# CVlab315/Domain-Adaptative-Hand-Pose-Estimation

Measured on AMD Instinct MI355X. Metric: images/sec (unique source+target images per A+B+C training iteration, 2*B*N/t_iter), higher is better.
Workload: dtype bf16; 1 GPU; RHD->H3D domain-adaptation iteration (steps A+B+C), resnet50 + 3-deconv neck + main head + 3 adversarial multiscale-fusion heads, 256x256, batch 64 source + 64 target per GPU, random init, synthetic batches; arch=resnet50, image_size=256, per_gpu_batch=64, global_batch=64, parallelism=dp1, hip_graphs=True, gradient_exchange=none (one rank)

## Files before the change

### domain-adaptative-hand-pose-estimation_amd/csrc/bn.hip

```cpp
#include "common.h"
#include "fp8_common.h"
#include <stdlib.h>
#include <string>

struct BnPlan { int cpr, TX, TY, colgroups, nslices, rows_per_slice; };

static BnPlan bn_plan(long rows, int C, int CH, long slice_cap_override = 0) {
  BnPlan p; p.cpr = C / CH;
  p.TX = p.cpr < 256 ? p.cpr : 256;
  while (256 % p.TX) --p.TX;
  p.TY = 256 / p.TX;
  p.colgroups = cdiv(p.cpr, p.TX);
  long want = rows / ((long)p.TY * 8); if (want < 1) want = 1;
  static const long slice_cap = getenv("MI355_BN_SLICES") ? atol(getenv("MI355_BN_SLICES")) : 1024;
  long cap = (slice_cap_override ? slice_cap_override : slice_cap) / p.colgroups; if (cap < 1) cap = 1;
  if (want > cap) want = cap;
  long rps = (rows + want - 1) / want; rps = ((rps + p.TY - 1) / p.TY) * p.TY;
  p.rows_per_slice = (int)rps; p.nslices = (int)((rows + rps - 1) / rps);
  return p;
}

static long bwd_slices() { static const long v = getenv("MI355_BN_BWD_SLICES") ? atol(getenv("MI355_BN_BWD_SLICES")) : 768; return v; }
extern "C" size_t mi355_bn_workspace(long rows, int C) {
  int ns = 0;
// ... 299 lines not shown
#pragma unroll
    for (int j = 0; j < 16; ++j) { s1 += q1[j]; s2 += q2[j]; }
  }
#pragma unroll
  for (int o = 32; o > 0; o >>= 1) { s1 += __shfl_down(s1, o, 64); s2 += __shfl_down(s2, o, 64); }
  if (lane != 0) return;
  if (dbeta) dbeta[c] = db0 + s1;
  if (dgamma) dgamma[c] = dg0 + s2;
  if (coeff) { coeff[c] = g * is; coeff[C + c] = s1 * inv_rows; coeff[2 * C + c] = s2 * inv_rows; }
}

template <typename T, int RELU, bool Q8 = false>
__global__ __launch_bounds__(256) void bn_bwd_apply_kernel(const T* __restrict__ dy, const T* __restrict__ x, const T* __restrict__ y,
                                                            const float* __restrict__ mean, const float* __restrict__ invstd,
                                                            const float* __restrict__ coeff, const float* __restrict__ beta,
                                                            T* __restrict__ dx, T* __restrict__ dres,
                                                            long rows, int C, int TX, const unsigned char* __restrict__ mask,
                                                            unsigned char* __restrict__ q8 = nullptr, float* __restrict__ q8_state = nullptr) {
  constexpr int CH = Chunk<T>::N;
  constexpr int relu = RELU;
  static_assert(!Q8 || CH == 8, "fp8 side output: bf16 gradients only");
  const int TY = 256 / TX;
  const int tx = threadIdx.x % TX, ty = threadIdx.x / TX;
  const int chunk = blockIdx.x * TX + tx;
  const bool colok = chunk * CH < C;
  if (!colok && !Q8) return;
  const int cpr = C / CH;
  float k0[CH], k1[CH], k2[CH], mu[CH], is[CH], sh[CH];
#pragma unroll
  for (int e = 0; e < CH; ++e) {
    const int c = colok ? chunk * CH + e : 0;
    k0[e] = coeff[c]; k1[e] = coeff[C + c]; k2[e] = coeff[2 * C + c]; mu[e] = mean[c]; is[e] = invstd[c];
    sh[e] = (relu == 2) ? beta[c] - mu[e] * k0[e] : 0.f;
  }
  float qscale = 0.f, amax = 0.f; unsigned seen = 0;
  if constexpr (Q8) { qscale = q8_state[0]; seen = fp8_amax_seen(q8_state); }
  auto finish = [&](size_t off, float (&g)[CH], float (&v)[CH], const float (&o)[CH], unsigned mb) {
    if (relu == 1) {
#pragma unroll
      for (int e = 0; e < CH; ++e) g[e] = o[e] > 0.f ? g[e] : 0.f; }
    else if (relu == 3) {
#pragma unroll
      for (int e = 0; e < CH; ++e) g[e] = ((mb >> e) & 1u) ? g[e] : 0.f; }
    else if (relu == 2) {
#pragma unroll
      for (int e = 0; e < CH; ++e) g[e] = (v[e] * k0[e] + sh[e]) > 0.f ? g[e] : 0.f; }
    if (dres) Chunk<T>::store(dres + off, g);
#pragma unroll
    for (int e = 0; e < CH; ++e) v[e] = k0[e] * (g[e] - k1[e] - (v[e] - mu[e]) * is[e] * k2[e]);
    Chunk<T>::store(dx + off, v);
    if constexpr (Q8) {
      float w[8];
#pragma unroll
      for (int e = 0; e < 8; ++e) { w[e] = (float)(T)v[e]; amax = fmaxf(amax, fabsf(w[e])); }
      const uint2 o = pack8_fp8<true>(w, qscale);
      const unsigned nx = __shfl_down(o.x, 1, 64), ny = __shfl_down(o.y, 1, 64);
      if ((tx & 1) == 0) *reinterpret_cast<uint4*>(q8 + off) = make_uint4(o.x, o.y, nx, ny);
    }
  };
  const long stride = (long)gridDim.y * TY;
  long r = colok ? (long)blockIdx.y * TY + ty : rows;
  for (; r + stride < rows; r += 2 * stride) {
    const size_t off0 = (size_t)r * C + (size_t)chunk * CH, off1 = (size_t)(r + stride) * C + (size_t)chunk * CH;
    float g0[CH], v0[CH], o0[CH], g1[CH], v1[CH], o1[CH];
    Chunk<T>::load(dy + off0, g0); Chunk<T>::load(x + off0, v0);
    Chunk<T>::load(dy + off1, g1); Chunk<T>::load(x + off1, v1);
    if (relu == 1) { Chunk<T>::load(y + off0, o0); Chunk<T>::load(y + off1, o1); }
    unsigned m0 = 0, m1 = 0;
    if (relu == 3) { m0 = mask[(size_t)r * cpr + chunk]; m1 = mask[(size_t)(r + stride) * cpr + chunk]; }
    finish(off0, g0, v0, o0, m0); finish(off1, g1, v1, o1, m1);
  }
  if (r < rows) {
    const size_t off = (size_t)r * C + (size_t)chunk * CH;
    float g[CH], v[CH], o[CH]; Chunk<T>::load(dy + off, g); Chunk<T>::load(x + off, v);
    if (relu == 1) Chunk<T>::load(y + off, o);
    finish(off, g, v, o, relu == 3 ? (unsigned)mask[(size_t)r * cpr + chunk] : 0u);
  }
  if constexpr (Q8) fp8_record_amax(amax, q8_state, seen);
}

struct BnResArgs {
  const void* dy; const void* x; const float* mean; const float* invstd; const float* gamma; const float* beta;
  void* dx; void* dres; float* dgamma; float* dbeta; const unsigned char* mask;
  float* partial;
  long rows; int C, G, R, rpb, keep, accumulate; float inv_rows;
  unsigned spin_limit;
};
#define BN_RES_MAXBLK 1024
#define BN_RES_KR 0
#define BN_RES_NT 1024
__device__ unsigned long long bn_res_sync[BN_RES_MAXBLK + 1];
__device__ unsigned bn_res_err[4];

__device__ __forceinline__ bool bn_res_grid_barrier(unsigned nblk, int t, unsigned spin_limit, int* ok_lds) {
  asm volatile("s_waitcnt vmcnt(0)" ::: "memory");
  __syncthreads();
  if (t == 0) {
    int ok = 1;
    unsigned long long* st = bn_res_sync + nblk;
    const unsigned long long v = __hip_atomic_fetch_add(st, 1ull, __ATOMIC_RELAXED, __HIP_MEMORY_SCOPE_AGENT);
    const unsigned long long target = (v / nblk + 1ull) * nblk;
    if (v + 1ull != target) {
      unsigned spins = 0;
      while (__hip_atomic_load(st, __ATOMIC_RELAXED, __HIP_MEMORY_SCOPE_AGENT) < target) {
        __builtin_amdgcn_s_sleep(4);
        if (++spins > spin_limit) {
          __hip_atomic_fetch_add(bn_res_err, 1u, __ATOMIC_RELAXED, __HIP_MEMORY_SCOPE_AGENT);
          ok = 0;
          break;
        }
      }
    }
    *ok_lds = ok;
  }
  __syncthreads();
  return *ok_lds != 0;
}

template <typename T, int RELU, int KR, int NT>
__global__ __launch_bounds__(NT) void bn_bwd_resident_kernel(BnResArgs p) {
  constexpr int CH = Chunk<T>::N, GC = 8 * CH, RL = NT / 8, NW = NT / 64, NL = NT / (GC * 2), RR = KR * RL;
  extern __shared__ __attribute__((aligned(16))) char smem[];
  const int t = threadIdx.x, tx = t & 7, ty = t >> 3, lane = t & 63, wave = t >> 6;
  const int g = blockIdx.x % p.G, r = blockIdx.x / p.G;
  const long row0 = (long)r * p.rpb;
  long row1 = row0 + p.rpb; if (row1 > p.rows) row1 = p.rows;
  const int nrows = row1 > row0 ? (int)(row1 - row0) : 0;
  const int keep = p.keep;
  uint4* xs = reinterpret_cast<uint4*>(smem);
  uint4* ds = xs + (size_t)keep * 8;
  float* red = reinterpret_cast<float*>(ds + (size_t)keep * 8);
  float* tot = red + NW * GC * 2;
  int* bar_ok = reinterpret_cast<int*>(tot + GC * 2);
  const T* __restrict__ X = reinterpret_cast<const T*>(p.x);
  const T* __restrict__ DY = reinterpret_cast<const T*>(p.dy);
  const int C = p.C, cpr = C / CH, c0 = g * GC + tx * CH, chunk = c0 / CH;
  float mu[CH], is[CH], sc[CH], sft[CH], s1[CH], s2[CH];
#pragma unroll
  for (int e = 0; e < CH; ++e) {
    mu[e] = p.mean[c0 + e]; is[e] = p.invstd[c0 + e]; s1[e] = 0.f; s2[e] = 0.f;
    sc[e] = p.gamma[c0 + e] * is[e];
    sft[e] = (RELU == 2) ? p.beta[c0 + e] - mu[e] * sc[e] : 0.f;
  }
  auto mask_of = [&](int lr) -> unsigned { return (RELU == 3) ? (unsigned)p.mask[(size_t)(row0 + lr) * cpr + chunk] : 0u; };
  auto fold = [&](const uint4& qxv, const uint4& qdv, unsigned mb) {
    float v[CH], gq[CH]; Chunk<T>::unpack(qxv, v); Chunk<T>::unpack(qdv, gq);
#pragma unroll
    for (int e = 0; e < CH; ++e) {
      if (RELU == 2) gq[e] = (v[e] * sc[e] + sft[e]) > 0.f ? gq[e] : 0.f;
      if (RELU == 3) gq[e] = ((mb >> e) & 1u) ? gq[e] : 0.f;
      s1[e] += gq[e]; s2[e] += gq[e] * ((v[e] - mu[e]) * is[e]);
    }
  };
  uint4 rx[KR > 0 ? KR : 1], rd[KR > 0 ? KR : 1];
  {
    unsigned mk[KR > 0 ? KR : 1];
#pragma unroll
    for (int k = 0; k < KR; ++k) {
      const int lr = ty + k * RL;
      rx[k] = make_uint4(0, 0, 0, 0); rd[k] = make_uint4(0, 0, 0, 0); mk[k] = 0;
      if (lr < nrows) {
        const size_t off = (size_t)(row0 + lr) * C + c0;
        rx[k] = *reinterpret_cast<const uint4*>(X + off); rd[k] = *reinterpret_cast<const uint4*>(DY + off); mk[k] = mask_of(lr);
      }
    }
#pragma unroll
    for (int k = 0; k < KR; ++k)
      if (ty + k * RL < nrows) fold(rx[k], rd[k], mk[k]);
  }
  for (int base = RR + ty; base < nrows; base += 4 * RL) {
    uint4 qx[4], qd[4]; unsigned mk[4];
#pragma unroll
    for (int k = 0; k < 4; ++k) {
      const int lr = base + k * RL;
      if (lr < nrows) {
        const size_t off = (size_t)(row0 + lr) * C + c0;
        qx[k] = *reinterpret_cast<const uint4*>(X + off); qd[k] = *reinterpret_cast<const uint4*>(DY + off); mk[k] = mask_of(lr);
      }
    }
#pragma unroll
    for (int k = 0; k < 4; ++k) {
      const int lr = base + k * RL, li = lr - RR;
      if (lr < nrows) {
        if (li < keep) { xs[li * 8 + tx] = qx[k]; ds[li * 8 + tx] = qd[k]; }
        fold(qx[k], qd[k], mk[k]);
      }
    }
  }
#pragma unroll
  for (int o = 8; o < 64; o <<= 1) {
#pragma unroll
    for (int e = 0; e < CH; ++e) { s1[e] += __shfl_xor(s1[e], o, 64); s2[e] += __shfl_xor(s2[e], o, 64); }
  }
  if (lane < 8) {
#pragma unroll
    for (int e = 0; e < CH; ++e) { red[(wave * GC + tx * CH + e) * 2] = s1[e]; red[(wave * GC + tx * CH + e) * 2 + 1] = s2[e]; }
  }
  __syncthreads();
  float* part = p.partial + ((size_t)g * p.R) * (GC * 2);
  if (t < GC * 2) {
    float a = 0.f;
#pragma unroll
    for (int w = 0; w < NW; ++w) a += red[w * GC * 2 + t];
    __hip_atomic_store(part + (size_t)r * (GC * 2) + t, a, __ATOMIC_RELAXED, __HIP_MEMORY_SCOPE_AGENT);
  }
  const bool exchanged = bn_res_grid_barrier((unsigned)(p.G * p.R), t, p.spin_limit, bar_ok);
  {
    const int i = t % (GC * 2), s = t / (GC * 2);
    const __amdgpu_buffer_rsrc_t rs = __builtin_amdgcn_make_buffer_rsrc(part, 0, (unsigned)(p.R * GC * 2 * 4), 0x00020000);
    float a = 0.f;
    for (int rr0 = s; rr0 < p.R; rr0 += 8 * NL) {
      float q[8];
#pragma unroll
      for (int k = 0; k < 8; ++k) {
        const int rr = rr0 + k * NL;
        q[k] = rr < p.R ? __uint_as_float(__builtin_amdgcn_raw_buffer_load_b32(rs, (rr * (GC * 2) + i) * 4, 0, 16)) : 0.f;
      }
#pragma unroll
      for (int k = 0; k < 8; ++k) a += q[k];
    }
    red[s * GC * 2 + i] = a;
  }
  __syncthreads();
  if (t < GC * 2) {
    float a = 0.f;
#pragma unroll
    for (int s = 0; s < NL; ++s) a += red[s * GC * 2 + t];
    tot[t] = a;
  }
  __syncthreads();
  float k1[CH], k2[CH];
#pragma unroll
  for (int e = 0; e < CH; ++e) {
    s1[e] = tot[(tx * CH + e) * 2]; s2[e] = tot[(tx * CH + e) * 2 + 1];
    if (!exchanged) { s1[e] = __builtin_nanf(""); s2[e] = __builtin_nanf(""); }
    k1[e] = s1[e] * p.inv_rows; k2[e] = s2[e] * p.inv_rows;
  }
  if (r == 0 && ty == 0) {
#pragma unroll
    for (int e = 0; e < CH; ++e) {
      if (p.dbeta) p.dbeta[c0 + e] = (p.accumulate ? p.dbeta[c0 + e] : 0.f) + s1[e];
      if (p.dgamma) p.dgamma[c0 + e] = (p.accumulate ? p.dgamma[c0 + e] : 0.f) + s2[e];
    }
  }
  T* __restrict__ DX = reinterpret_cast<T*>(p.dx);
  T* __restrict__ DR = reinterpret_cast<T*>(p.dres);
  auto finish = [&](int lr, const uint4& qxv, const uint4& qdv, unsigned mb) {
    const size_t off = (size_t)(row0 + lr) * C + c0;
    float v[CH], gq[CH]; Chunk<T>::unpack(qxv, v); Chunk<T>::unpack(qdv, gq);
#pragma unroll
    for (int e = 0; e < CH; ++e) {
      if (RELU == 2) gq[e] = (v[e] * sc[e] + sft[e]) > 0.f ? gq[e] : 0.f;
      if (RELU == 3) gq[e] = ((mb >> e) & 1u) ? gq[e] : 0.f;
    }
    if (DR) Chunk<T>::store(DR + off, gq);
#pragma unroll
    for (int e = 0; e < CH; ++e) v[e] = sc[e] * (gq[e] - k1[e] - (v[e] - mu[e]) * is[e] * k2[e]);
    Chunk<T>::store(DX + off, v);
  };
#pragma unroll
  for (int k = 0; k < KR; ++k) {
    const int lr = ty + k * RL;
    if (lr < nrows) finish(lr, rx[k], rd[k], mask_of(lr));
  }
  const int nlds = nrows - RR < keep ? nrows - RR : keep;
  for (int li = ty; li < nlds; li += RL) finish(RR + li, xs[li * 8 + tx], ds[li * 8 + tx], mask_of(RR + li));
  for (int base = RR + keep + ty; base < nrows; base += 4 * RL) {
    uint4 qx[4], qd[4]; unsigned mk[4];
#pragma unroll
    for (int k = 0; k < 4; ++k) {
      const int lr = base + k * RL;
      if (lr < nrows) {
        const size_t off = (size_t)(row0 + lr) * C + c0;
        qx[k] = *reinterpret_cast<const uint4*>(X + off); qd[k] = *reinterpret_cast<const uint4*>(DY + off); mk[k] = mask_of(lr);
      }
    }
#pragma unroll
    for (int k = 0; k < 4; ++k) {
      const int lr = base + k * RL;
      if (lr < nrows) finish(lr, qx[k], qd[k], mk[k]);
    }
  }
}

template <typename T>
__global__ __launch_bounds__(256) void apply_relu_mask_kernel(T* __restrict__ g, const unsigned char* __restrict__ mask, size_t nchunks) {
  constexpr int CH = Chunk<T>::N;
  for (size_t i = (size_t)blockIdx.x * 256 + threadIdx.x; i < nchunks; i += (size_t)gridDim.x * 256) {
    float v[CH]; Chunk<T>::load(g + i * CH, v);
    const unsigned mb = mask[i];
#pragma unroll
    for (int e = 0; e < CH; ++e) v[e] = ((mb >> e) & 1u) ? v[e] : 0.f;
    Chunk<T>::store(g + i * CH, v);
  }
}

template <typename T>
__global__ __launch_bounds__(256) void bn_relu_maxpool_kernel(const T* __restrict__ x, const float* __restrict__ scale_shift, T* __restrict__ y,
                                                               uint8_t* __restrict__ arg, int N, int H, int W, int C, int Ho, int Wo) {
  constexpr int CH = Chunk<T>::N;
  const int cpr = C / CH;
  const unsigned total = (unsigned)N * Ho * Wo * cpr;
  for (unsigned id = blockIdx.x * 256u + threadIdx.x; id < total; id += gridDim.x * 256u) {
    const int ch = (int)(id % (unsigned)cpr); unsigned r = id / (unsigned)cpr;
    const int ox = (int)(r % (unsigned)Wo); r /= (unsigned)Wo; const int oy = (int)(r % (unsigned)Ho); const int n = (int)(r / (unsigned)Ho);
    float sc[CH], sh[CH], best[CH]; int bi[CH]; bool first = true;
#pragma unroll
    for (int e = 0; e < CH; ++e) { sc[e] = scale_shift[ch * CH + e]; sh[e] = scale_shift[C + ch * CH + e]; best[e] = -INFINITY; bi[e] = 0; }
    for (int kh = 0; kh < 3; ++kh) {
      const int iy = 2 * oy - 1 + kh; if (iy < 0 || iy >= H) continue;
      for (int kw = 0; kw < 3; ++kw) {
        const int ix = 2 * ox - 1 + kw; if (ix < 0 || ix >= W) continue;
        float v[CH]; Chunk<T>::load(x + (((size_t)n * H + iy) * W + ix) * C + (size_t)ch * CH, v);
        const int code = kh * 3 + kw;
#pragma unroll
        for (int e = 0; e < CH; ++e) {
          float u = v[e] * sc[e] + sh[e];
          u = u < 0.f ? 0.f : u;
          u = (float)(T)u;
          if (first) bi[e] = code;
          if (u > best[e] || u != u) { best[e] = u; bi[e] = code; }
        }
        first = false;
      }
    }
    const size_t o = (((size_t)n * Ho + oy) * Wo + ox) * C + (size_t)ch * CH;
    Chunk<T>::store(y + o, best);
    store_bytes<CH>(arg + o, bi);
  }
}

__global__ __launch_bounds__(256) void colsum_finalize_kernel(const float* __restrict__ partial, int nslices, int C, float* out, int accumulate) {
  const int lane = threadIdx.x & 63;
  const int c = blockIdx.x * 4 + (threadIdx.x >> 6);
  if (c >= C) return;
  float q[16];
#pragma unroll
  for (int j = 0; j < 16; ++j) { const int i = lane + 64 * j; q[j] = (i < nslices) ? partial[((size_t)i * C + c) * 2] : 0.f; }
  float s = 0.f;
#pragma unroll
  for (int j = 0; j < 16; ++j) s += q[j];
#pragma unroll
  for (int o = 32; o > 0; o >>= 1) s += __shfl_down(s, o, 64);
  if (lane == 0) out[c] = (accumulate ? out[c] : 0.f) + s;
}

static int q8_check(const void* q8_out, const float* q8_state, int dtype, int C) {
  if (!q8_out && !q8_state) return 0;
  if (!q8_out || !q8_state || dtype != MI355_BF16 || C % 16) MI_FAIL(MI355_EINVAL, "bn: the fp8 side output needs both q8 pointers, bf16 activations and C %% 16 == 0");
  return 0;
}
static int bn_check(long rows, int C, int dtype, int* CH) {
  if (dtype != MI355_F32 && dtype != MI355_BF16) MI_FAIL(MI355_EINVAL, "bn: bad dtype");
  *CH = dtype == MI355_BF16 ? 8 : 4;
  if (rows < 1 || C < 1 || C % *CH) MI_FAIL(MI355_EINVAL, "bn: C=%d must be a positive multiple of %d (rows=%ld)", C, *CH, rows);
  return 0;
}
static dim3 apply_grid(const BnPlan& p, long rows, bool backward = false) {
  long gy = rows / ((long)p.TY * 4); if (gy < 1) gy = 1;
  static const long fwd_cap = getenv("MI355_BN_APPLY_CAP") ? atol(getenv("MI355_BN_APPLY_CAP")) : 2048;
  static const long bwd_cap = getenv("MI355_BN_BWD_CAP") ? atol(getenv("MI355_BN_BWD_CAP")) : 1024;
  long cap = (backward ? bwd_cap : fwd_cap) / p.colgroups; if (cap < 1) cap = 1;
  if (gy > cap) gy = cap;
  return dim3(p.colgroups, (unsigned)gy);
}
// ... 45 lines not shown
  if (stat_updates < 0 || stat_updates > 8) MI_FAIL(MI355_EINVAL, "bn_train_fwd_partials: stat_updates=%d", stat_updates);
  if (!partial || nslices < 1 || !scale_shift) MI_FAIL(MI355_EINVAL, "bn_train_fwd_partials: partial / scale_shift missing");
  hipStream_t st = as_stream(stream);
  BnPlan p = bn_plan(rows, C, CH);
  static const int wide_min = getenv("MI355_BN_WIDE_FINALIZE") ? atoi(getenv("MI355_BN_WIDE_FINALIZE")) : 512;
  const double nb = (double)rows * C * (dtype == MI355_BF16 ? 2.0 : 4.0);
  char lab[96];
  if (prof_on()) snprintf(lab, sizeof(lab), "rows%ld C%d ns%d%s%s", rows, C, nslices, relu ? " relu" : "", residual ? " +res" : "");
  {
    ProfScope ps(st, 0.0, 12.0 * nslices * C, 1, prof_on() ? (std::string("bn_finalize ") + lab).c_str() : nullptr);
    if (nslices >= wide_min) hipLaunchKernelGGL(bn_finalize_wide_kernel, dim3(C), dim3(256), 0, st, partial, nslices, C, gamma, beta, running_mean, running_var, nbt, save_mean, save_invstd, scale_shift, eps, momentum, stat_updates);
    else hipLaunchKernelGGL(bn_finalize_kernel, dim3(cdiv(C, 4)), dim3(256), 0, st, partial, nslices, C, gamma, beta, running_mean, running_var, nbt, save_mean, save_invstd, scale_shift, eps, momentum, stat_updates);
  }
  dim3 ga = apply_grid(p, rows);
  const float* nf = nullptr;
  ProfScope ps(st, 0.0, nb * (residual ? 3 : 2), 1, prof_on() ? (std::string("bn_apply ") + lab).c_str() : nullptr);
  if (q8_out) hipLaunchKernelGGL((bn_apply_kernel<bf16_t, false, true>), ga, dim3(256), 0, st, (const bf16_t*)x, (const bf16_t*)residual, (bf16_t*)y, (const float*)scale_shift, nf, nf, nf, nf, eps, rows, C, p.TX, relu, mk, (unsigned char*)q8_out, q8_state);
  else if (dtype == MI355_BF16) hipLaunchKernelGGL((bn_apply_kernel<bf16_t, false>), ga, dim3(256), 0, st, (const bf16_t*)x, (const bf16_t*)residual, (bf16_t*)y, (const float*)scale_shift, nf, nf, nf, nf, eps, rows, C, p.TX, relu, mk);
  else hipLaunchKernelGGL((bn_apply_kernel<float, false>), ga, dim3(256), 0, st, (const float*)x, (const float*)residual, (float*)y, (const float*)scale_shift, nf, nf, nf, nf, eps, rows, C, p.TX, relu, mk);
  MI_CHECK_LAUNCH("bn_train_fwd_partials");
  return MI355_OK;
}

extern "C" int mi355_bn_relu_maxpool_fwd_partials(const void* x, void* y_pool, uint8_t* argidx, const float* gamma, const float* beta,
                                                  float* running_mean, float* running_var, int64_t* nbt, float* save_mean,
                                                  float* save_invstd, int N, int H, int W, int C, float eps, float momentum,
                                                  int stat_updates, int dtype, const float* partial, int nslices, float* scale_shift,
                                                  void* stream) {
  const long rows = (long)N * H * W;
  int CH; if (int e = bn_check(rows, C, dtype, &CH)) return e;
  if (stat_updates < 0 || stat_updates > 8) MI_FAIL(MI355_EINVAL, "bn_relu_maxpool_fwd_partials: stat_updates=%d", stat_updates);
  if (!partial || nslices < 1 || !scale_shift || !argidx || !y_pool) MI_FAIL(MI355_EINVAL, "bn_relu_maxpool_fwd_partials: null argument");
  if (rows * (C / CH) >= (1L << 31)) MI_FAIL(MI355_EINVAL, "bn_relu_maxpool_fwd_partials: %ld chunks exceed the kernel's 32-bit index: split the batch", rows * (C / CH));
  hipStream_t st = as_stream(stream);
  static const int wide_min = getenv("MI355_BN_WIDE_FINALIZE") ? atoi(getenv("MI355_BN_WIDE_FINALIZE")) : 512;
  char lab[96];
  if (prof_on()) snprintf(lab, sizeof(lab), "rows%ld C%d ns%d", rows, C, nslices);
  {
    ProfScope ps(st, 0.0, 12.0 * nslices * C, 1, prof_on() ? (std::string("bn_finalize ") + lab).c_str() : nullptr);
    if (nslices >= wide_min) hipLaunchKernelGGL(bn_finalize_wide_kernel, dim3(C), dim3(256), 0, st, partial, nslices, C, gamma, beta, running_mean, running_var, nbt, save_mean, save_invstd, scale_shift, eps, momentum, stat_updates);
    else hipLaunchKernelGGL(bn_finalize_kernel, dim3(cdiv(C, 4)), dim3(256), 0, st, partial, nslices, C, gamma, beta, running_mean, running_var, nbt, save_mean, save_invstd, scale_shift, eps, momentum, stat_updates);
  }
  const int Ho = (H + 2 - 3) / 2 + 1, Wo = (W + 2 - 3) / 2 + 1;
  const long total = (long)N * Ho * Wo * (C / CH);
  int grid = (int)((total + 255) / 256); if (grid > 8192) grid = 8192;
  ProfScope ps(st, 0.0, (double)rows * C * (dtype == MI355_BF16 ? 2.0 : 4.0) * 1.25, 1, prof_on() ? (std::string("bn_relu_maxpool ") + lab).c_str() : nullptr);
  if (dtype == MI355_BF16) hipLaunchKernelGGL(bn_relu_maxpool_kernel<bf16_t>, dim3(grid), dim3(256), 0, st, (const bf16_t*)x, (const float*)scale_shift, (bf16_t*)y_pool, argidx, N, H, W, C, Ho, Wo);
  else hipLaunchKernelGGL(bn_relu_maxpool_kernel<float>, dim3(grid), dim3(256), 0, st, (const float*)x, (const float*)scale_shift, (float*)y_pool, argidx, N, H, W, C, Ho, Wo);
  MI_CHECK_LAUNCH("bn_relu_maxpool_fwd_partials");
  return MI355_OK;
}

extern "C" int mi355_bn_eval_fwd(const void* x, const void* residual, void* y, const float* gamma, const float* beta,
                                 const float* running_mean, const float* running_var, long rows, int C, float eps, int relu,
                                 int dtype, void* stream) {
  int CH; if (int e = bn_check(rows, C, dtype, &CH)) return e;
  hipStream_t st = as_stream(stream);
  BnPlan p = bn_plan(rows, C, CH);
  dim3 ga = apply_grid(p, rows);
  const float* nf = nullptr;
  if (dtype == MI355_BF16) hipLaunchKernelGGL((bn_apply_kernel<bf16_t, true>), ga, dim3(256), 0, st, (const bf16_t*)x, (const bf16_t*)residual, (bf16_t*)y, nf, gamma, beta, running_mean, running_var, eps, rows, C, p.TX, relu, (unsigned char*)nullptr);
  else hipLaunchKernelGGL((bn_apply_kernel<float, true>), ga, dim3(256), 0, st, (const float*)x, (const float*)residual, (float*)y, nf, gamma, beta, running_mean, running_var, eps, rows, C, p.TX, relu, (unsigned char*)nullptr);
  MI_CHECK_LAUNCH("bn_eval_fwd");
  return MI355_OK;
}

struct BnResPlan { int G, R, rpb, keep; size_t lds, max_lds; };
static int g_bn_resident = -1;
extern "C" int mi355_bn_set_resident(int on) {
  const int prev = g_bn_resident;
  g_bn_resident = on < 0 ? -1 : (on ? 1 : 0);
  return prev;
}
static bool bn_resident_plan(long rows, int C, int CH, BnResPlan* q) {
  static const bool env_on = !(getenv("MI355_BN_RESIDENT") && atoi(getenv("MI355_BN_RESIDENT")) == 0);
  if (g_bn_resident == 0 || (g_bn_resident < 0 && !env_on)) return false;
  static int ncu = 0; static size_t max_lds = 0;
  if (!ncu) {
    int dev = 0, v = 0;
    if (hipGetDevice(&dev) != hipSuccess) return false;
    if (hipDeviceGetAttribute(&v, hipDeviceAttributeMaxSharedMemoryPerBlock, dev) != hipSuccess) return false;
    max_lds = (size_t)v;
    if (hipDeviceGetAttribute(&v, hipDeviceAttributeMultiprocessorCount, dev) != hipSuccess) return false;
    ncu = v > 256 ? 256 : v;
  }
  const int GC = 8 * CH;
  if (C % GC) return false;
  static const long min_bytes = getenv("MI355_BN_RESIDENT_MIN") ? atol(getenv("MI355_BN_RESIDENT_MIN")) : 0;
  if (rows * C * (16 / CH) < min_bytes) return false;
  q->G = C / GC;
  if (q->G > ncu) return false;
  long R = ncu / q->G; if (R > rows) R = rows;
  q->rpb = (int)((rows + R - 1) / R);
  q->R = (int)((rows + q->rpb - 1) / q->rpb);
  static const long max_bytes = getenv("MI355_BN_RESIDENT_MAX") ? atol(getenv("MI355_BN_RESIDENT_MAX")) : (1L << 62);
  if (rows * C * (16 / CH) > max_bytes) return false;
  const size_t scratch = (size_t)(BN_RES_NT / 64 * GC * 2 + GC * 2 + 4) * sizeof(float);
  long keep = (long)((max_lds - scratch) / 256);
  const long reg_rows = (long)BN_RES_KR * (BN_RES_NT / 8);
  const long rest = q->rpb > reg_rows ? q->rpb - reg_rows : 0;
  if (keep > rest) keep = rest;
  q->keep = (int)keep;
  q->lds = (size_t)keep * 256 + scratch;
  q->max_lds = max_lds;
  return (size_t)q->G * q->R <= (size_t)ncu && q->G * q->R <= BN_RES_MAXBLK;
}
static unsigned g_bn_res_spin = 1u << 19;
extern "C" int mi355_bn_resident_set_spin_limit(unsigned limit) {
  g_bn_res_spin = limit ? limit : (1u << 19);
  return MI355_OK;
}
#define BN_RES_NOT_RESIDENT 1
template <typename T, int RELU>
static int bn_resident_launch(const BnResArgs& a, size_t lds, size_t max_lds, hipStream_t st) {
  static int fits = -1;
  auto kern = bn_bwd_resident_kernel<T, RELU, BN_RES_KR, BN_RES_NT>;
  if (fits < 0) {
    if (hipFuncSetAttribute(reinterpret_cast<const void*>(kern), hipFuncAttributeMaxDynamicSharedMemorySize, (int)max_lds) != hipSuccess)
      MI_FAIL(MI355_ELAUNCH, "bn_bwd: cannot raise the dynamic LDS limit to %zu bytes", max_lds);
    int nb = 0;
    if (hipOccupancyMaxActiveBlocksPerMultiprocessor(&nb, kern, BN_RES_NT, max_lds) != hipSuccess) nb = 0;
    fits = nb >= 1 ? 1 : 0;
  }
  if (!fits) return BN_RES_NOT_RESIDENT;
  hipLaunchKernelGGL(kern, dim3(a.G * a.R), dim3(BN_RES_NT), lds, st, a);
  return MI355_OK;
}
extern "C" int mi355_bn_resident_timeouts(unsigned* out) {
  unsigned v[4] = {0, 0, 0, 0};
  if (!out) MI_FAIL(MI355_EINVAL, "bn_resident_timeouts: out is null");
  if (hipMemcpyFromSymbol(v, HIP_SYMBOL(bn_res_err), sizeof(v)) != hipSuccess) MI_FAIL(MI355_ELAUNCH, "bn_resident_timeouts: copy failed");
  *out = v[0];
  return MI355_OK;
}
extern "C" int mi355_bn_resident_reset(void) {
  static const unsigned long long zeros[BN_RES_MAXBLK + 1] = {0};
  static const unsigned zerr[4] = {0, 0, 0, 0};
  if (hipDeviceSynchronize() != hipSuccess) MI_FAIL(MI355_ELAUNCH, "bn_resident_reset: device synchronize failed");
  if (hipMemcpyToSymbol(HIP_SYMBOL(bn_res_sync), zeros, sizeof(zeros)) != hipSuccess ||
      hipMemcpyToSymbol(HIP_SYMBOL(bn_res_err), zerr, sizeof(zerr)) != hipSuccess) MI_FAIL(MI355_ELAUNCH, "bn_resident_reset: copy failed");
  return MI355_OK;
}

static void launch_bwd_apply(int dtype, int relu, dim3 ga, hipStream_t st, const void* dy, const void* x, const void* y, const float* save_mean,
                             const float* save_invstd, const float* coeff, const float* beta, void* dx, void* dresidual, long rows, int C,
                             int TX, const unsigned char* mk, void* q8_out, float* q8_state) {
#define MI_APP(T, R) hipLaunchKernelGGL((bn_bwd_apply_kernel<T, R>), ga, dim3(256), 0, st, (const T*)dy, (const T*)x, (const T*)y, save_mean, save_invstd, coeff, beta, (T*)dx, (T*)dresidual, rows, C, TX, mk)
#define MI_APQ(R) hipLaunchKernelGGL((bn_bwd_apply_kernel<bf16_t, R, true>), ga, dim3(256), 0, st, (const bf16_t*)dy, (const bf16_t*)x, (const bf16_t*)y, save_mean, save_invstd, coeff, beta, (bf16_t*)dx, (bf16_t*)dresidual, rows, C, TX, mk, (unsigned char*)q8_out, q8_state)
#define MI_APP4(T) do { if (relu == 0) MI_APP(T, 0); else if (relu == 1) MI_APP(T, 1); else if (relu == 2) MI_APP(T, 2); else MI_APP(T, 3); } while (0)
  if (q8_out) { if (relu == 0) MI_APQ(0); else if (relu == 1) MI_APQ(1); else if (relu == 2) MI_APQ(2); else MI_APQ(3); }
  else if (dtype == MI355_BF16) MI_APP4(bf16_t); else MI_APP4(float);
#undef MI_APP4
#undef MI_APQ
#undef MI_APP
}

extern "C" int mi355_bn_bwd(const void* dy, const void* x, const void* y, const float* gamma, const float* beta, const float* save_mean,
                            const float* save_invstd, void* dx, void* dresidual, float* dgamma, float* dbeta, int accumulate,
                            long rows, int C, int relu, int dtype, void* ws, size_t ws_bytes, const void* relu_mask, void* q8_out,
                            float* q8_state, void* stream) {
  int CH; if (int e = bn_check(rows, C, dtype, &CH)) return e;
  if (!ws || ws_bytes < mi355_bn_workspace(rows, C)) MI_FAIL(MI355_EWORKSPACE, "bn_bwd: workspace too small");
  const unsigned char* mk = reinterpret_cast<const unsigned char*>(relu_mask);
  if (relu) relu = mk ? 3 : (y ? 1 : 2);
  if (relu == 2 && !beta) MI_FAIL(MI355_EINVAL, "bn_bwd: relu without y needs beta");
  hipStream_t st = as_stream(stream);
  BnResPlan rp;
  if (relu != 1 && !q8_out && bn_resident_plan(rows, C, CH, &rp)) {
    if (ws_bytes < (size_t)rp.G * rp.R * (8 * CH) * 2 * sizeof(float)) MI_FAIL(MI355_EWORKSPACE, "bn_bwd: workspace too small for the one-launch partials");
    BnResArgs a;
    a.dy = dy; a.x = x; a.mean = save_mean; a.invstd = save_invstd; a.gamma = gamma; a.beta = beta; a.dx = dx; a.dres = dresidual;
    a.dgamma = dgamma; a.dbeta = dbeta; a.mask = mk; a.partial = reinterpret_cast<float*>(ws); a.rows = rows; a.C = C;
    a.G = rp.G; a.R = rp.R; a.rpb = rp.rpb; a.keep = rp.keep; a.accumulate = accumulate; a.inv_rows = 1.0f / (float)rows;
    a.spin_limit = g_bn_res_spin;
    int e;
    char lab[112];
    if (prof_on()) snprintf(lab, sizeof(lab), "bn_bwd_res rows%ld C%d relu%d%s keep%d/%d", rows, C, relu, dresidual ? " +dres" : "", rp.keep, rp.rpb);
    ProfScope ps(st, 0.0, (double)rows * C * (dtype == MI355_BF16 ? 2.0 : 4.0) * (dresidual ? 4 : 3), 1, prof_on() ? lab : nullptr);
    if (dtype == MI355_BF16) e = relu == 0 ? bn_resident_launch<bf16_t, 0>(a, rp.lds, rp.max_lds, st) : relu == 2 ? bn_resident_launch<bf16_t, 2>(a, rp.lds, rp.max_lds, st) : bn_resident_launch<bf16_t, 3>(a, rp.lds, rp.max_lds, st);
    else e = relu == 0 ? bn_resident_launch<float, 0>(a, rp.lds, rp.max_lds, st) : relu == 2 ? bn_resident_launch<float, 2>(a, rp.lds, rp.max_lds, st) : bn_resident_launch<float, 3>(a, rp.lds, rp.max_lds, st);
    if (e == MI355_OK) { MI_CHECK_LAUNCH("bn_bwd (resident)"); return MI355_OK; }
    if (e != BN_RES_NOT_RESIDENT) return e;
  }
  BnPlan p = bn_plan(rows, C, CH, bwd_slices());
  float* partial = reinterpret_cast<float*>(ws);
  float* coeff = partial + (size_t)p.nslices * C * 3;
  dim3 g(p.colgroups, p.nslices);
#define MI_RED(T, R) hipLaunchKernelGGL((bn_bwd_reduce_kernel<T, true, R>), g, dim3(256), 0, st, (const T*)dy, (const T*)x, (const T*)y, save_mean, save_invstd, gamma, beta, partial, rows, C, p.TX, p.rows_per_slice, mk)
#define MI_RED4(T) do { if (relu == 0) MI_RED(T, 0); else if (relu == 1) MI_RED(T, 1); else if (relu == 2) MI_RED(T, 2); else MI_RED(T, 3); } while (0)
  const double nb = (double)rows * C * (dtype == MI355_BF16 ? 2.0 : 4.0);
  char lab[96];
  if (prof_on()) snprintf(lab, sizeof(lab), "rows%ld C%d relu%d%s", rows, C, relu, dresidual ? " +dres" : "");
  {
    ProfScope ps(st, 0.0, nb * 2, 1, prof_on() ? (std::string("bn_bwd_reduce ") + lab).c_str() : nullptr);
    if (dtype == MI355_BF16) MI_RED4(bf16_t); else MI_RED4(float);
  }
#undef MI_RED4
#undef MI_RED
  {
    ProfScope ps(st, 0.0, 12.0 * p.nslices * C, 1, prof_on() ? (std::string("bn_bwd_finalize ") + lab).c_str() : nullptr);
    hipLaunchKernelGGL(bn_bwd_finalize_kernel, dim3(cdiv(C, 4)), dim3(256), 0, st, partial, p.nslices, C, 1.0f / (float)rows, gamma, save_invstd, dgamma, dbeta, accumulate, coeff);
  }
  dim3 ga = apply_grid(p, rows, true);
  if (int e = q8_check(q8_out, q8_state, dtype, C)) return e;
  ProfScope ps(st, 0.0, nb * (dresidual ? 4 : 3), 1, prof_on() ? (std::string("bn_bwd_apply ") + lab).c_str() : nullptr);
  launch_bwd_apply(dtype, relu, ga, st, dy, x, y, save_mean, save_invstd, coeff, beta, dx, dresidual, rows, C, p.TX, mk, q8_out, q8_state);
  MI_CHECK_LAUNCH("bn_bwd");
  return MI355_OK;
}

extern "C" int mi355_bn_bwd_partials(const void* dy, const void* x, const void* y, const float* gamma, const float* beta,
                                     const float* save_mean, const float* save_invstd, void* dx, void* dresidual, float* dgamma,
                                     float* dbeta, int accumulate, long rows, int C, int relu, int dtype, const float* partial,
                                     int nslices, float* coeff, const void* relu_mask, void* q8_out, float* q8_state, void* stream) {
  int CH; if (int e = bn_check(rows, C, dtype, &CH)) return e;
  if (!partial || nslices < 1 || !coeff) MI_FAIL(MI355_EINVAL, "bn_bwd_partials: partial / coeff missing");
  const unsigned char* mk = reinterpret_cast<const unsigned char*>(relu_mask);
  if (relu) relu = mk ? 3 : (y ? 1 : 2);
  if (relu == 2 && !beta) MI_FAIL(MI355_EINVAL, "bn_bwd_partials: relu without y needs beta");
  hipStream_t st = as_stream(stream);
  BnPlan p = bn_plan(rows, C, CH);
  hipLaunchKernelGGL(bn_bwd_finalize_kernel, dim3(cdiv(C, 4)), dim3(256), 0, st, partial, nslices, C, 1.0f / (float)rows, gamma, save_invstd, dgamma, dbeta, accumulate, coeff);
  dim3 ga = apply_grid(p, rows, true);
  if (int e = q8_check(q8_out, q8_state, dtype, C)) return e;
  launch_bwd_apply(dtype, relu, ga, st, dy, x, y, save_mean, save_invstd, coeff, beta, dx, dresidual, rows, C, p.TX, mk, q8_out, q8_state);
  MI_CHECK_LAUNCH("bn_bwd_partials");
  return MI355_OK;
}

extern "C" int mi355_apply_relu_mask(void* g, const void* relu_mask, long rows, int C, int dtype, void* stream) {
  int CH; if (int e = bn_check(rows, C, dtype, &CH)) return e;
  if (!g || !relu_mask) MI_FAIL(MI355_EINVAL, "apply_relu_mask: null pointer");
  const size_t nchunks = (size_t)rows * (C / CH);
  long grid = (long)((nchunks + 255) / 256); if (grid > 4096) grid = 4096;
  if (dtype == MI355_BF16) hipLaunchKernelGGL(apply_relu_mask_kernel<bf16_t>, dim3((unsigned)grid), dim3(256), 0, as_stream(stream), (bf16_t*)g, (const unsigned char*)relu_mask, nchunks);
  else hipLaunchKernelGGL(apply_relu_mask_kernel<float>, dim3((unsigned)grid), dim3(256), 0, as_stream(stream), (float*)g, (const unsigned char*)relu_mask, nchunks);
  MI_CHECK_LAUNCH("apply_relu_mask");
  return MI355_OK;
}

extern "C" int mi355_colsum(const void* dy, float* out, long rows, int C, int dtype, int accumulate, void* ws, size_t ws_bytes,
                            void* stream) {
  int CH; if (int e = bn_check(rows, C, dtype, &CH)) return e;
  if (!ws || ws_bytes < mi355_colsum_workspace(rows, C)) MI_FAIL(MI355_EWORKSPACE, "colsum: workspace too small");
  hipStream_t st = as_stream(stream);
  BnPlan p = bn_plan(rows, C, CH);
  float* partial = reinterpret_cast<float*>(ws);
  dim3 g(p.colgroups, p.nslices);
  if (dtype == MI355_BF16) hipLaunchKernelGGL((bn_bwd_reduce_kernel<bf16_t, false, 0>), g, dim3(256), 0, st, (const bf16_t*)dy, (const bf16_t*)nullptr, (const bf16_t*)nullptr, (const float*)nullptr, (const float*)nullptr, (const float*)nullptr, (const float*)nullptr, partial, rows, C, p.TX, p.rows_per_slice, (const unsigned char*)nullptr);
  else hipLaunchKernelGGL((bn_bwd_reduce_kernel<float, false, 0>), g, dim3(256), 0, st, (const float*)dy, (const float*)nullptr, (const float*)nullptr, (const float*)nullptr, (const float*)nullptr, (const float*)nullptr, (const float*)nullptr, partial, rows, C, p.TX, p.rows_per_slice, (const unsigned char*)nullptr);
  hipLaunchKernelGGL(colsum_finalize_kernel, dim3(cdiv(C, 4)), dim3(256), 0, st, partial, p.nslices, C, out, accumulate);
  MI_CHECK_LAUNCH("colsum");
  return MI355_OK;
}
```

Before: 4305 images/s.

## Replace BN backward grid barrier with tagged partial publication and per-slot polling

The resident BN backward kernel no longer runs a global atomic counter barrier followed by a read of partials. Each block now publishes its per-channel partial sums as 64-bit words that pair the value with a launch tag. Readers poll those slots directly until every tag matches, so a block only waits for the partials it actually needs. A completion counter per grid size advances the tag from one launch to the next. This drops the serialized atomic barrier and the workspace partials, at the cost of static global scratch, a 256-block cap, and tag/epoch logic that has to stay correct across graph replays. Optional timestamp instrumentation and profiling scripts are also added.

```diff
diff --git a/domain-adaptative-hand-pose-estimation_amd/csrc/bn.hip b/domain-adaptative-hand-pose-estimation_amd/csrc/bn.hip
--- a/domain-adaptative-hand-pose-estimation_amd/csrc/bn.hip
+++ b/domain-adaptative-hand-pose-estimation_amd/csrc/bn.hip
@@ -405,40 +405,29 @@
 struct BnResArgs {
   const void* dy; const void* x; const float* mean; const float* invstd; const float* gamma; const float* beta;
   void* dx; void* dres; float* dgamma; float* dbeta; const unsigned char* mask;
-  float* partial;
   long rows; int C, G, R, rpb, keep, accumulate; float inv_rows;
   unsigned spin_limit;
 };
-#define BN_RES_MAXBLK 1024
+#define BN_RES_MAXBLK 256
+#define BN_RES_GRAN 128
+#define BN_RES_SW 8
 #define BN_RES_KR 0
 #define BN_RES_NT 1024
-__device__ unsigned long long bn_res_sync[BN_RES_MAXBLK + 1];
+__device__ unsigned long long bn_res_gran[BN_RES_MAXBLK * BN_RES_GRAN];
+__device__ unsigned bn_res_done[2][BN_RES_MAXBLK + 1];
 __device__ unsigned bn_res_err[4];
-
-__device__ __forceinline__ bool bn_res_grid_barrier(unsigned nblk, int t, unsigned spin_limit, int* ok_lds) {
-  asm volatile("s_waitcnt vmcnt(0)" ::: "memory");
-  __syncthreads();
-  if (t == 0) {
-    int ok = 1;
-    unsigned long long* st = bn_res_sync + nblk;
-    const unsigned long long v = __hip_atomic_fetch_add(st, 1ull, __ATOMIC_RELAXED, __HIP_MEMORY_SCOPE_AGENT);
-    const unsigned long long target = (v / nblk + 1ull) * nblk;
-    if (v + 1ull != target) {
-      unsigned spins = 0;
-      while (__hip_atomic_load(st, __ATOMIC_RELAXED, __HIP_MEMORY_SCOPE_AGENT) < target) {
-        __builtin_amdgcn_s_sleep(4);
-        if (++spins > spin_limit) {
-          __hip_atomic_fetch_add(bn_res_err, 1u, __ATOMIC_RELAXED, __HIP_MEMORY_SCOPE_AGENT);
-          ok = 0;
-          break;
-        }
-      }
-    }
-    *ok_lds = ok;
-  }
-  __syncthreads();
-  return *ok_lds != 0;
-}
+static_assert(BN_RES_MAXBLK == 256, "a launch adds 256 to its completion count and the tag keeps 8 bits of n - 1");
+
+#ifdef BN_RES_STAMPS
+__device__ unsigned long long bn_res_stamp[BN_RES_MAXBLK * 8];
+#define BN_STAMP(k) do { __builtin_amdgcn_sched_barrier(0); if (t == 0) bn_res_stamp[blockIdx.x * 8 + (k)] = wall_clock64(); \
+                         __builtin_amdgcn_sched_barrier(0); } while (0)
+extern "C" int mi355_bn_resident_stamps(unsigned long long* out) {
+  return hipMemcpyFromSymbol(out, HIP_SYMBOL(bn_res_stamp), sizeof(unsigned long long) * BN_RES_MAXBLK * 8) == hipSuccess ? MI355_OK : MI355_ELAUNCH;
+}
+#else
+#define BN_STAMP(k) do {} while (0)
+#endif
 
 template <typename T, int RELU, int KR, int NT>
 __global__ __launch_bounds__(NT) void bn_bwd_resident_kernel(BnResArgs p) {
@@ -453,11 +442,17 @@
   uint4* xs = reinterpret_cast<uint4*>(smem);
   uint4* ds = xs + (size_t)keep * 8;
   float* red = reinterpret_cast<float*>(ds + (size_t)keep * 8);
-  float* tot = red + NW * GC * 2;
+  float* grp = red + NW * GC * 2;
+  float* tot = grp + NL * GC * 2;
   int* bar_ok = reinterpret_cast<int*>(tot + GC * 2);
   const T* __restrict__ X = reinterpret_cast<const T*>(p.x);
   const T* __restrict__ DY = reinterpret_cast<const T*>(p.dy);
   const int C = p.C, cpr = C / CH, c0 = g * GC + tx * CH, chunk = c0 / CH;
+  BN_STAMP(0);
+  const unsigned nblk = (unsigned)(p.G * p.R);
+  unsigned* done = &bn_res_done[GC * 2 == BN_RES_GRAN ? 1 : 0][nblk];
+  const unsigned tag = 0x80000000u | (GC * 2 == BN_RES_GRAN ? 0x40000000u : 0u) | ((nblk - 1u) << 22) |
+                       ((__hip_atomic_load(done, __ATOMIC_RELAXED, __HIP_MEMORY_SCOPE_AGENT) >> 8) & 0x3fffffu);
   float mu[CH], is[CH], sc[CH], sft[CH], s1[CH], s2[CH];
 #pragma unroll
   for (int e = 0; e < CH; ++e) {
@@ -519,39 +514,54 @@
 #pragma unroll
     for (int e = 0; e < CH; ++e) { red[(wave * GC + tx * CH + e) * 2] = s1[e]; red[(wave * GC + tx * CH + e) * 2 + 1] = s2[e]; }
   }
-  __syncthreads();
-  float* part = p.partial + ((size_t)g * p.R) * (GC * 2);
-  if (t < GC * 2) {
-    float a = 0.f;
-#pragma unroll
-    for (int w = 0; w < NW; ++w) a += red[w * GC * 2 + t];
-    __hip_atomic_store(part + (size_t)r * (GC * 2) + t, a, __ATOMIC_RELAXED, __HIP_MEMORY_SCOPE_AGENT);
-  }
-  const bool exchanged = bn_res_grid_barrier((unsigned)(p.G * p.R), t, p.spin_limit, bar_ok);
-  {
-    const int i = t % (GC * 2), s = t / (GC * 2);
-    const __amdgpu_buffer_rsrc_t rs = __builtin_amdgcn_make_buffer_rsrc(part, 0, (unsigned)(p.R * GC * 2 * 4), 0x00020000);
-    float a = 0.f;
-    for (int rr0 = s; rr0 < p.R; rr0 += 8 * NL) {
-      float q[8];
-#pragma unroll
-      for (int k = 0; k < 8; ++k) {
-        const int rr = rr0 + k * NL;
-        q[k] = rr < p.R ? __uint_as_float(__builtin_amdgcn_raw_buffer_load_b32(rs, (rr * (GC * 2) + i) * 4, 0, 16)) : 0.f;
-      }
-#pragma unroll
-      for (int k = 0; k < 8; ++k) a += q[k];
-    }
-    red[s * GC * 2 + i] = a;
-  }
+  if (t == 0) *bar_ok = 1;
+  BN_STAMP(1);
   __syncthreads();
   if (t < GC * 2) {
     float a = 0.f;
 #pragma unroll
-    for (int s = 0; s < NL; ++s) a += red[s * GC * 2 + t];
+    for (int w = 0; w < NW; ++w) a += red[w * GC * 2 + t];
+    __hip_atomic_store(bn_res_gran + (size_t)blockIdx.x * BN_RES_GRAN + t, ((unsigned long long)tag << 32) | __float_as_uint(a),
+                       __ATOMIC_RELAXED, __HIP_MEMORY_SCOPE_AGENT);
+  }
+  BN_STAMP(2);
+  {
+    const int i = t % (GC * 2), s = t / (GC * 2);
+    const __amdgpu_buffer_rsrc_t rs = __builtin_amdgcn_make_buffer_rsrc(bn_res_gran, 0, (unsigned)sizeof(bn_res_gran), 0x00020000);
+    float a = 0.f;
+    bool arrived = true;
+    for (int rr0 = s; rr0 < p.R && arrived; rr0 += BN_RES_SW * NL) {
+      float q[BN_RES_SW];
+      for (unsigned spins = 0;;) {
+        asm volatile("" ::: "memory");
+        bool ok = true;
+#pragma unroll
+        for (int k = 0; k < BN_RES_SW; ++k) {
+          const int rr = rr0 + k * NL;
+          const auto gv = __builtin_amdgcn_raw_buffer_load_b64(rs, rr < p.R ? ((rr * p.G + g) * BN_RES_GRAN + i) * 8 : 0x7ffffff0, 0, 16);
+          q[k] = rr < p.R ? __uint_as_float(gv[0]) : 0.f; ok &= (gv[1] == tag) | (rr >= p.R);
+        }
+        if (__all(ok)) break;
+        if (++spins > p.spin_limit) { arrived = false; break; }
+        __builtin_amdgcn_s_sleep(4);
+      }
+#pragma unroll
+      for (int k = 0; k < BN_RES_SW; ++k) a += q[k];
+    }
+    grp[s * GC * 2 + i] = a;
+    if (!arrived && lane == 0) *bar_ok = 0;
+  }
+  __syncthreads();
+  const bool exchanged = *bar_ok != 0;
+  if (!exchanged && t == 0) __hip_atomic_fetch_add(bn_res_err, 1u, __ATOMIC_RELAXED, __HIP_MEMORY_SCOPE_AGENT);
+  if (t < GC * 2) {
+    float a = 0.f;
+#pragma unroll
+    for (int s = 0; s < NL; ++s) a += grp[s * GC * 2 + t];
     tot[t] = a;
   }
   __syncthreads();
+  BN_STAMP(3);
   float k1[CH], k2[CH];
 #pragma unroll
   for (int e = 0; e < CH; ++e) {
@@ -568,6 +578,9 @@
   }
   T* __restrict__ DX = reinterpret_cast<T*>(p.dx);
   T* __restrict__ DR = reinterpret_cast<T*>(p.dres);
+#ifdef BN_RES_STAMPS
+  bool stamped = false;
+#endif
   auto finish = [&](int lr, const uint4& qxv, const uint4& qdv, unsigned mb) {
     const size_t off = (size_t)(row0 + lr) * C + c0;
     float v[CH], gq[CH]; Chunk<T>::unpack(qxv, v); Chunk<T>::unpack(qdv, gq);
@@ -580,6 +593,9 @@
 #pragma unroll
     for (int e = 0; e < CH; ++e) v[e] = sc[e] * (gq[e] - k1[e] - (v[e] - mu[e]) * is[e] * k2[e]);
     Chunk<T>::store(DX + off, v);
+#ifdef BN_RES_STAMPS
+    if (!stamped) { BN_STAMP(4); stamped = true; }
+#endif
   };
 #pragma unroll
   for (int k = 0; k < KR; ++k) {
@@ -604,6 +620,8 @@
       if (lr < nrows) finish(lr, qx[k], qd[k], mk[k]);
     }
   }
+  if (t == 0) __hip_atomic_fetch_add(done, blockIdx.x == 0 ? (unsigned)BN_RES_MAXBLK + 1u - nblk : 1u, __ATOMIC_RELAXED, __HIP_MEMORY_SCOPE_AGENT);
+  BN_STAMP(5);
 }
 
 template <typename T>
@@ -815,7 +833,7 @@
     if (hipDeviceGetAttribute(&v, hipDeviceAttributeMaxSharedMemoryPerBlock, dev) != hipSuccess) return false;
     max_lds = (size_t)v;
     if (hipDeviceGetAttribute(&v, hipDeviceAttributeMultiprocessorCount, dev) != hipSuccess) return false;
-    ncu = v > 256 ? 256 : v;
+    ncu = v > BN_RES_MAXBLK ? BN_RES_MAXBLK : v;
   }
   const int GC = 8 * CH;
   if (C % GC) return false;
@@ -828,7 +846,7 @@
   q->R = (int)((rows + q->rpb - 1) / q->rpb);
   static const long max_bytes = getenv("MI355_BN_RESIDENT_MAX") ? atol(getenv("MI355_BN_RESIDENT_MAX")) : (1L << 62);
   if (rows * C * (16 / CH) > max_bytes) return false;
-  const size_t scratch = (size_t)(BN_RES_NT / 64 * GC * 2 + GC * 2 + 4) * sizeof(float);
+  const size_t scratch = (size_t)(BN_RES_NT / 64 * GC * 2 + BN_RES_NT + GC * 2 + 4) * sizeof(float);
   long keep = (long)((max_lds - scratch) / 256);
   const long reg_rows = (long)BN_RES_KR * (BN_RES_NT / 8);
   const long rest = q->rpb > reg_rows ? q->rpb - reg_rows : 0;
@@ -867,11 +885,14 @@
   return MI355_OK;
 }
 extern "C" int mi355_bn_resident_reset(void) {
-  static const unsigned long long zeros[BN_RES_MAXBLK + 1] = {0};
+  static const unsigned zdone[2][BN_RES_MAXBLK + 1] = {{0}};
   static const unsigned zerr[4] = {0, 0, 0, 0};
+  void* gran = nullptr;
   if (hipDeviceSynchronize() != hipSuccess) MI_FAIL(MI355_ELAUNCH, "bn_resident_reset: device synchronize failed");
-  if (hipMemcpyToSymbol(HIP_SYMBOL(bn_res_sync), zeros, sizeof(zeros)) != hipSuccess ||
+  if (hipGetSymbolAddress(&gran, HIP_SYMBOL(bn_res_gran)) != hipSuccess || hipMemset(gran, 0, sizeof(bn_res_gran)) != hipSuccess ||
+      hipMemcpyToSymbol(HIP_SYMBOL(bn_res_done), zdone, sizeof(zdone)) != hipSuccess ||
       hipMemcpyToSymbol(HIP_SYMBOL(bn_res_err), zerr, sizeof(zerr)) != hipSuccess) MI_FAIL(MI355_ELAUNCH, "bn_resident_reset: copy failed");
+  if (hipDeviceSynchronize() != hipSuccess) MI_FAIL(MI355_ELAUNCH, "bn_resident_reset: device synchronize failed");
   return MI355_OK;
 }
 
@@ -900,10 +921,9 @@
   hipStream_t st = as_stream(stream);
   BnResPlan rp;
   if (relu != 1 && !q8_out && bn_resident_plan(rows, C, CH, &rp)) {
-    if (ws_bytes < (size_t)rp.G * rp.R * (8 * CH) * 2 * sizeof(float)) MI_FAIL(MI355_EWORKSPACE, "bn_bwd: workspace too small for the one-launch partials");
     BnResArgs a;
     a.dy = dy; a.x = x; a.mean = save_mean; a.invstd = save_invstd; a.gamma = gamma; a.beta = beta; a.dx = dx; a.dres = dresidual;
-    a.dgamma = dgamma; a.dbeta = dbeta; a.mask = mk; a.partial = reinterpret_cast<float*>(ws); a.rows = rows; a.C = C;
+    a.dgamma = dgamma; a.dbeta = dbeta; a.mask = mk; a.rows = rows; a.C = C;
     a.G = rp.G; a.R = rp.R; a.rpb = rp.rpb; a.keep = rp.keep; a.accumulate = accumulate; a.inv_rows = 1.0f / (float)rows;
     a.spin_limit = g_bn_res_spin;
     int e;
diff --git a/profiles/bn_exchange_anatomy.py b/profiles/bn_exchange_anatomy.py
--- /dev/null
+++ b/profiles/bn_exchange_anatomy.py
@@ -0,0 +1,93 @@
+import argparse
+import ctypes
+import os
+import sys
+
+import numpy as np
+import torch
+
+ROOT = os.path.dirname(os.path.dirname(os.path.abspath(__file__)))
+sys.path.insert(0, os.path.join(ROOT, 'domain-adaptative-hand-pose-estimation_amd'))
+
+GEOMS = [(262144, 256, 2), (262144, 256, 3), (65536, 512, 3), (16384, 256, 2), (16384, 1024, 3), (65536, 256, 2), (262144, 64, 2),
+         (65536, 128, 2), (4096, 2048, 3), (1048576, 64, 2), (4096, 512, 2), (262144, 128, 2), (16384, 512, 2)]
+PHASES = [('pass 1', 0, 1), ('fold+publish', 1, 2), ('exchange', 2, 3), ('to 1st store', 3, 4), ('pass 2', 4, 5), ('kernel', 0, 5)]
+
+
+def blocks_of(rows, C, group_channels=64, ncu=256):
+    G = C // group_channels
+    R = min(ncu // G, rows)
+    rpb = -(-rows // R)
+    return G, -(-rows // rpb)
+
+
+def make_case(rows, C, mode, dtype, dev, seed):
+    from mi355 import ops
+    g = torch.Generator(device=dev).manual_seed(seed)
+    N, H, W = (rows // 4096, 64, 64) if rows >= 4096 else (1, 1, rows)
+    x, dy = ops.nhwc_empty(N, C, H, W, dtype, dev), ops.nhwc_empty(N, C, H, W, dtype, dev)
+    x.permute(0, 2, 3, 1).copy_(torch.randn(N, H, W, C, generator=g, device=dev))
+    dy.permute(0, 2, 3, 1).copy_(torch.randn(N, H, W, C, generator=g, device=dev))
+    ch = 8 if dtype == torch.bfloat16 else 4
+    case = dict(x=x, dy=dy, gamma=1 + 0.1 * torch.randn(C, generator=g, device=dev), beta=0.1 * torch.randn(C, generator=g, device=dev),
+                mean=0.1 * torch.randn(C, generator=g, device=dev), invstd=1 + 0.1 * torch.rand(C, generator=g, device=dev), mask=None, mode=mode)
+    if mode == 3:
+        case['mask'] = torch.randint(0, 256, (rows * C // ch,), generator=g, device=dev, dtype=torch.uint8)
+    return case
+
+
+def run_case(case, want_dres):
+    from mi355 import ops
+    C = case['x'].shape[1]
+    dg, db = torch.zeros(C, device=case['x'].device), torch.zeros(C, device=case['x'].device)
+    dx, dres = ops.bn_bwd(case['dy'], case['x'], None, case['gamma'], case['mean'], case['invstd'], dg, db, False, True, want_dres,
+                          beta=case['beta'], relu_mask=case['mask'])
+    return dx, dres, dg, db
+
+
+def main():
+    ap = argparse.ArgumentParser()
+    ap.add_argument('--reps', type=int, default=7)
+    ap.add_argument('--label', default=os.path.basename(os.environ.get('MI355_LIB', 'default library')))
+    a = ap.parse_args()
+    import mi355
+    from mi355 import ops
+    lib = mi355.load()
+    if not hasattr(lib, 'mi355_bn_resident_stamps'):
+        sys.exit('this library has no stamps: build it with --flags "-DBN_RES_STAMPS" and point MI355_LIB at it')
+    lib.mi355_bn_resident_stamps.restype, lib.mi355_bn_resident_stamps.argtypes = ctypes.c_int, [ctypes.c_void_p]
+    lib.mi355_bn_set_resident(1)
+    dev = torch.device('cuda:0')
+    evict = torch.empty(512 << 20, dtype=torch.uint8, device=dev)
+    buf = np.zeros((256, 8), dtype=np.uint64)
+    print('== %s: bn_bwd_resident_kernel by in-kernel stamps, us; median / max over blocks x %d launches behind a cache-evicting fill' % (a.label, a.reps))
+    print('%-22s %5s | %s | %13s | %13s' % ('geometry', 'grid', ' | '.join('%13s' % n for n, _, _ in PHASES), 'publish skew', 'last pub -> 3'))
+    for rows, C, mode in GEOMS:
+        case = make_case(rows, C, mode, torch.bfloat16, dev, 1)
+        G, R = blocks_of(rows, C)
+        n = G * R
+        run_case(case, mode == 3)
+        torch.cuda.synchronize()
+        spans = {name: [] for name, _, _ in PHASES}
+        skew, net = [], []
+        for _ in range(a.reps):
+            evict.fill_(1)
+            run_case(case, mode == 3)
+            torch.cuda.synchronize()
+            if lib.mi355_bn_resident_stamps(buf.ctypes.data) != 0:
+                sys.exit('reading the stamps failed')
+            s = buf[:n].astype(np.int64) * 0.01
+            for name, i, j in PHASES:
+                spans[name].extend(s[:, j] - s[:, i])
+            skew.append(s[:, 2].max() - s[:, 2].min())
+            net.extend(s[:, 3] - s[:, 2].max())
+        cells = ['%6.2f /%6.2f' % (np.median(spans[name]), np.max(spans[name])) for name, _, _ in PHASES]
+        print('%-22s %5d | %s | %6.2f /%6.2f | %6.2f /%6.2f' % ('rows%d C%d relu%d' % (rows, C, mode), n, ' | '.join(cells),
+                                                              np.median(skew), np.max(skew), np.median(net), np.max(net)))
+        del case
+    if ops.bn_resident_timeouts():
+        sys.exit('a block gave up: the figures above are void')
+
+
+if __name__ == '__main__':
+    main()
diff --git a/profiles/bn_exchange_bits.py b/profiles/bn_exchange_bits.py
--- /dev/null
+++ b/profiles/bn_exchange_bits.py
@@ -0,0 +1,69 @@
+import hashlib
+import json
+import os
+import subprocess
+import sys
+
+HERE = os.path.dirname(os.path.abspath(__file__))
+sys.path.insert(0, HERE)
+
+F32 = [(16384, 256, 2), (4096, 512, 3)]
+
+
+def digest(t):
+    if t is None:
+        return '-'
+    import torch
+    return hashlib.sha256(t.contiguous().view(torch.uint8).cpu().numpy().tobytes()).hexdigest()
+
+
+def worker():
+    import torch
+    import bn_exchange_anatomy as an
+    import mi355
+    from mi355 import ops
+    mi355.load().mi355_bn_set_resident(1)
+    dev = torch.device('cuda:0')
+    out = {}
+    cases = [(g, torch.bfloat16) for g in an.GEOMS] + [(g, torch.float32) for g in F32]
+    for seed, ((rows, C, mode), dt) in enumerate(cases):
+        case = an.make_case(rows, C, mode, dt, dev, 1000 + seed)
+        for rep in range(2):
+            dx, dres, dg, db = an.run_case(case, mode == 3)
+            torch.cuda.synchronize()
+            key = 'rows%d C%d relu%d %s #%d' % (rows, C, mode, 'bf16' if dt == torch.bfloat16 else 'f32', rep)
+            out[key] = [digest(dx.permute(0, 2, 3, 1)), digest(dg), digest(db), digest(dres.permute(0, 2, 3, 1) if dres is not None else None)]
+        del case, dx, dres
+    out['timeouts'] = ops.bn_resident_timeouts()
+    print('BITS ' + json.dumps(out))
+
+
+def main():
+    if len(sys.argv) == 2 and sys.argv[1] == '--worker':
+        return worker()
+    if len(sys.argv) != 3:
+        sys.exit(__doc__)
+    res = []
+    for lib in sys.argv[1:]:
+        env = dict(os.environ, MI355_LIB=os.path.abspath(lib))
+        r = subprocess.run([sys.executable, os.path.abspath(__file__), '--worker'], env=env, capture_output=True, text=True, timeout=600)
+        line = [l for l in r.stdout.splitlines() if l.startswith('BITS ')]
+        if r.returncode != 0 or not line:
+            sys.exit('worker for %s failed (%d):\n%s' % (lib, r.returncode, r.stderr[-3000:]))
+        res.append(json.loads(line[-1][5:]))
+    a, b = res
+    ta, tb = a.pop('timeouts'), b.pop('timeouts')
+    print('A = %s\nB = %s\nSHA-256 of the raw bytes, first 12 hex digits; give-ups: A %d, B %d' % (sys.argv[1], sys.argv[2], ta, tb))
+    print('%-34s %-6s %-14s %-14s' % ('case (#: launch)', '', 'A', 'B'))
+    bad = ta + tb
+    for key in a:
+        for name, da, db in zip(('dx', 'dgamma', 'dbeta', 'dres'), a[key], b[key]):
+            same = da == db
+            bad += not same
+            print('%-34s %-6s %-14s %-14s %s' % (key, name, da[:12], db[:12], 'equal' if same else 'DIFFERENT'))
+    print('%d of %d outputs differ' % (bad, 4 * len(a)))
+    sys.exit(1 if bad else 0)
+
+
+if __name__ == '__main__':
+    main()
```

After: 4383 images/s (median of 6 runs). +1.8%, better.
